# daooshee/ReReVST-Code

Hardware: AMD Instinct MI355X
Metric: stylized frames/sec at 512x512, 1 style (higher is better)
Workload: dtype f32

## Files before the change

rerevst-code_amd/csrc/conv_ups5.h:

```cpp
#pragma once

struct Ups5Tab {
    static constexpr int G2[5][3] = {{2, 0, 0}, {1, 1, 1}, {-1, -1, 1}, {-1, 1, 1}, {0, 0, 2}};
    static constexpr int BT4[4][4] = {{1, 0, -1, 0}, {0, 1, 1, 0}, {0, -1, 1, 0}, {0, -1, 0, 1}};
    static constexpr int AT[4][5] = {{1, 1, 0, -1, 0}, {0, 1, 1, 0, 0}, {0, 1, 0, 1, 0}, {0, 1, -1, 0, 1}};
    static constexpr int DS[5] = {0, 1, 2, 2, 3};
};
template <int T, int R>
constexpr int ups5_coef(int k) { return T == 0 ? Ups5Tab::BT4[R][k] : Ups5Tab::AT[R][k]; }
template <int T, int R, int N>
__device__ __forceinline__ f32x4 ups5_comb(const f32x4 (&x)[N]) {
    constexpr int F = [] { for (int k = 0; k < N; ++k) if (ups5_coef<T, R>(k) == 1) return k; return -1; }();
    static_assert(F >= 0, "every row has a +1 coefficient");
    f32x4 r = x[F];
    static_for([&](auto kc) {
        constexpr int k = decltype(kc)::value;
        constexpr int c = ups5_coef<T, R>(k);
        static_assert(c == 0 || c == 1 || c == -1, "0 / +-1 coefficients");
        if constexpr (k != F && c == 1) r = e4add(r, x[k]);
        else if constexpr (c == -1) r = f4sub(r, x[k]);
    }, std::make_integer_sequence<int, N>{});
    return r;
}

struct Ups5Geo {
    static constexpr int NT = 256, NB = 2;
    static constexpr int NPOS = 29;
    static constexpr int NUB = 26;
    static constexpr int NPIECE = 16;
    static constexpr int HALO = 18, HALF = 18 * 9;
    static constexpr int PIECES = HALO * HALO * 4;
    static constexpr int RAW_IT = (PIECES + NT - 1) / NT;
    static constexpr int RAW_BYTES = RAW_IT * NT * 16;
    static constexpr int U_BYTES = NUB * 32 * 16 * 4;
    static constexpr int U_IT = U_BYTES / 16 / NT;
    static_assert(U_IT * NT * 16 == U_BYTES, "U image is a whole number of LDS-DMA rounds");
    static constexpr int SMEM = 2 * RAW_BYTES + 2 * U_BYTES + WINO_PAR_BYTES;
    static_assert(SMEM <= 160 * 1024, "LDS");
    static constexpr int OCC = 1;
    static constexpr int vidx(int i) { return i < 25 ? Ups5Tab::DS[i % 5] * 4 + Ups5Tab::DS[i / 5] : (i == 25 ? 5 : i == 26 ? 9 : i == 27 ? 6 : 10); }
    static constexpr int issued(int j) { return (j + 2 < NUB ? 2 : 0) + (j < NPIECE ? 1 : 0); }
    static constexpr int younger(int i) {
        return i == 0 ? 2 + issued(0) : i == 1 ? issued(0) + issued(1) : (i - 2 < NPIECE ? 1 : 0) + issued(i - 1) + issued(i);
    }
    static constexpr int col_iter(int dx) { return 4 * dx + 6; }
    static constexpr int row_iter(int r) { return col_iter(3) + 1 + r; }
};
static_assert(Ups5Geo::row_iter(3) < Ups5Geo::NPOS, "next chunk transformed inside the MFMA loop");

template <int EPI, int PERIMG>
__device__ __forceinline__ void conv_ups5_body(const ConvP& p) {
    static_assert(!(EPI & (E_POOL | E_RES | E_RES_UPS | E_NORM2)), "conv1 epilogues only: bias, activation, saved-stat normalise");
    using G = Ups5Geo;
    constexpr int RAW_BYTES = G::RAW_BYTES, U_BYTES = G::U_BYTES, NT = G::NT, NB = G::NB, NPOS = G::NPOS, NUB = G::NUB;
    extern __shared__ __attribute__((aligned(16))) char smem[];
    const int tid = threadIdx.x;
    const int wave = __builtin_amdgcn_readfirstlane(tid >> 6);
    const int lane = tid & 63, t = lane & 15, q = lane >> 4;
    const int tr = t >> 3, tc = t & 7;
    const int tg = wave;
    const int nchunks = p.Cin >> 4;
    const int n_ntiles = p.Cout >> 5;

    struct Item { int tx, ty, b, nt; };
    Item cur, nxt, dlt;
    {
        const int GD = gridDim.x, w = blockIdx.x;
        int pix, dpix;
        if (p.xcd_slabs) {
            const int PT = (GD >> 3) / n_ntiles;
            pix = (w & 7) * PT + (w >> 3) / n_ntiles; dpix = 8 * PT;
            cur.nt = (w >> 3) % n_ntiles; dlt.nt = 0;
        } else {
            cur.nt = w % n_ntiles; pix = w / n_ntiles;
            dlt.nt = GD % n_ntiles; dpix = GD / n_ntiles;
        }
        cur.tx = pix % p.tiles_x; cur.ty = (pix / p.tiles_x) % p.tiles_y; cur.b = pix / (p.tiles_x * p.tiles_y);
        dlt.tx = dpix % p.tiles_x; dlt.ty = (dpix / p.tiles_x) % p.tiles_y; dlt.b = dpix / (p.tiles_x * p.tiles_y);
    }
    auto advance = [&](const Item& a) {
        Item r = a;
        r.nt += dlt.nt;
        int carry = 0;
        if (r.nt >= n_ntiles) { r.nt -= n_ntiles; carry = 1; }
        r.tx += dlt.tx + carry;
        if (r.tx >= p.tiles_x) { r.tx -= p.tiles_x; r.ty += 1; }
        r.ty += dlt.ty;
        if (r.ty >= p.tiles_y) { r.ty -= p.tiles_y; r.b += 1; }
        r.b += dlt.b;
        return r;
    };
    auto in_of = [&](const Item& a) {
        return p.in + (size_t)a.b * (size_t)(p.Hi + 2) * (p.Wi + 2) * p.Cin + (size_t)(((a.ty + p.ty0) * 16) * (p.Wi + 2) + (a.tx + p.tx0) * 16) * p.Cin;
    };
    auto w_of = [&](const Item& a) { return p.wpk + (size_t)a.nt * nchunks * (NUB * 32 * 16); };
    int asrc[G::RAW_IT];
#pragma unroll
    for (int it = 0; it < G::RAW_IT; ++it) {
        const int e = it * NT + tid;
        int P = e >> 2;
        const int qq = e & 3;
        if (P >= G::HALO * G::HALO) P = 0;
        const int hf = P >= G::HALF, rem = P - hf * G::HALF;
        const int hy = rem / 9, hx = 2 * (rem - hy * 9) + hf;
        asrc[it] = ((hy * (p.Wi + 2) + hx) * p.Cin + 4 * (qq ^ ((hx >> 1) & 3))) * 4;
    }
    const int raw_last_num = ((G::RAW_IT - 1) * NT + wave * 64 < G::PIECES) ? 0x7fffffff : 0;
    bool have = cur.b < p.B, have_nxt = false;
    const float* in_t = in_of(cur);
    const float* w_t = w_of(cur);
    const float* in_n = in_t;
    const float* w_n = w_t;
    auto stage_u = [&](int chunk) {
        char* udst = smem + 2 * RAW_BYTES + (chunk & 1) * U_BYTES;
#pragma unroll
        for (int it = 0; it < G::U_IT; ++it) bufld16(w_t, udst + (it * NT + wave * 64) * 16, tid * 16, chunk * U_BYTES + it * NT * 16);
    };
    auto stage_raw = [&](int chunk) {
        char* rdst = smem + (chunk & 1) * RAW_BYTES;
#pragma unroll
        for (int it = 0; it < G::RAW_IT; ++it)
            if (it * NT + wave * 64 < G::PIECES) bufld16(in_t, rdst + (it * NT + wave * 64) * 16, asrc[it], chunk * 64);
    };
    char* const par = smem + 2 * RAW_BYTES + 2 * U_BYTES;
    auto stage_params = [&](int ntile, int img) {
        if (wave < 2) {
            const int e = tid;
            const int row = e >> 3, col = (e & 7) * 4;
            const float* src = p.bias;
            const int pb = PERIMG ? img * p.par_bstride : 0;
            int off = ntile * 32 + col;
            if (row >= 1 && row <= 4) { src = (EPI & E_NORM1) ? p.n1 : p.bias; off = (EPI & E_NORM1) ? ntile * 32 + col + pb + (row - 1) * p.Cout : off; }
            if (row > 4) { src = p.bias; off = ntile * 32; }
            glds16(src + off, par + wave * 1024);
        }
    };

    const unsigned lds0 = (unsigned)(size_t)(__attribute__((address_space(3))) char*)smem;
    unsigned offD[4];
#pragma unroll
    for (int dx = 0; dx < 4; ++dx) {
        const int hy = 4 * tg + 2 * tr, hx = 2 * tc + dx;
        const int P = (hx & 1) * G::HALF + hy * 9 + (hx >> 1);
        offD[dx] = lds0 + P * 64 + ((q ^ ((hx >> 1) & 3)) << 4);
    }
    const unsigned offU = lds0 + 2 * RAW_BYTES + t * 64 + ((q ^ ((0 - (t >> 2)) & 3)) << 4);
    const unsigned offU1 = offU + U_BYTES;

    f32x4 acc[NPOS][NB];
    f32x4 va[16], vb[16];
    auto pass = [](f32x4& x0, f32x4& x1, f32x4& x2, f32x4& x3) {
        const f32x4 a[4] = {x0, x1, x2, x3};
        x0 = ups5_comb<0, 0>(a); x1 = ups5_comb<0, 1>(a); x2 = ups5_comb<0, 2>(a); x3 = ups5_comb<0, 3>(a);
    };
    auto col_pass = [&](f32x4 (&d)[16], int dx) { pass(d[dx * 4 + 0], d[dx * 4 + 1], d[dx * 4 + 2], d[dx * 4 + 3]); };
    auto row_pass = [&](f32x4 (&d)[16], int r) { pass(d[0 * 4 + r], d[1 * 4 + r], d[2 * 4 + r], d[3 * 4 + r]); };

    auto chunk_body = [&](int c, auto par_c, auto first_c, f32x4 (&vcur)[16], f32x4 (&vnext)[16]) {
        constexpr int PAR = decltype(par_c)::value;
        constexpr bool FIRST = decltype(first_c)::value;
        const bool own_u = c + 1 < nchunks, own_r = c + 2 < nchunks;
        const rsrc_t rs_u = make_rsrc(own_u ? w_t : w_n);
        const rsrc_t rs_r = make_rsrc(own_r ? in_t : in_n);
        const rsrc_t rs_rl = make_rsrc(own_r ? in_t : in_n, raw_last_num);
        const int usoff = own_u ? (c + 1) * U_BYTES : 0;
        const int rsoff = (own_r ? c + 2 : c + 2 - nchunks) * 64;
        char* const udst = smem + 2 * RAW_BYTES + (1 - PAR) * U_BYTES;
        char* const rdst = smem + PAR * RAW_BYTES;
        const unsigned ub = PAR ? offU1 : offU;
        constexpr int RB = (1 - PAR) * RAW_BYTES;
        f32x4 u[4][NB];
        f32x4 (&d)[16] = vnext;
        u[0][0] = lds_rd128<0>(ub);
        u[0][1] = lds_rd128<1024>(ub);
        u[1][0] = lds_rd128<2048>(ub);
        u[1][1] = lds_rd128<2048 + 1024>(ub);
        static_for([&](auto ic) {
            constexpr int i = decltype(ic)::value;
            if constexpr (i + 2 < NUB) {
                u[(i + 2) & 3][0] = lds_rd128<(i + 2) * 2048>(ub);
                u[(i + 2) & 3][1] = lds_rd128<(i + 2) * 2048 + 1024>(ub);
            }
            if constexpr (i < 16) d[i] = lds_rd128<RB + (i & 3) * 576>(offD[i >> 2]);
            constexpr int US = (i < NUB ? i : NUB - 1) & 3;
            if constexpr (i < NUB) {
                constexpr int cdx = (i - 6) / 4;
                if constexpr (i >= 6 && (i - 6) % 4 == 0 && cdx < 4) {
                    static_assert(G::col_iter(cdx) == i, "column release schedule");
                    asm volatile("s_waitcnt lgkmcnt(%6)" : "+v"(d[cdx * 4 + 0]), "+v"(d[cdx * 4 + 1]), "+v"(d[cdx * 4 + 2]), "+v"(d[cdx * 4 + 3]),
                                 "+v"(u[US][0]), "+v"(u[US][1]) : "i"(G::younger(i)));
                } else {
                    lds_release2<G::younger(i)>(u[US][0], u[US][1]);
                }
            }
            __builtin_amdgcn_sched_barrier(0);
            if constexpr (i < G::U_IT) bufld16_rs(rs_u, udst + (i * NT + wave * 64) * 16, tid * 16, usoff + i * NT * 16);
            if constexpr (i < G::RAW_IT) bufld16_rs(i == G::RAW_IT - 1 ? rs_rl : rs_r, rdst + (i * NT + wave * 64) * 16, asrc[i], rsoff);
            const f32x4 vv = vcur[G::vidx(i)];
#pragma unroll
            for (int s = 0; s < 4; ++s)
#pragma unroll
                for (int nb = 0; nb < NB; ++nb)
                    acc[i][nb] = __builtin_amdgcn_mfma_f32_16x16x4f32(u[US][nb][s], vv[s], (FIRST && s == 0) ? f32x4{0.f, 0.f, 0.f, 0.f} : acc[i][nb], 0, 0, 0);
            static_for([&](auto xc) {
                constexpr int k = decltype(xc)::value;
                if constexpr (G::col_iter(k) == i) col_pass(d, k);
                if constexpr (G::row_iter(k) == i) row_pass(d, k);
            }, std::make_integer_sequence<int, 4>{});
        }, std::make_integer_sequence<int, NPOS>{});
    };

    int par_ntile = -1, par_img = -1;
    if (have) {
        stage_raw(0);
        stage_u(0);
        stage_raw(1);
        stage_params(cur.nt, cur.b);
        par_ntile = cur.nt; par_img = cur.b;
        __syncthreads();
#pragma unroll
        for (int k = 0; k < 16; ++k) va[k] = *(const f32x4*)(smem + (offD[k >> 2] - lds0) + (k & 3) * 576);
#pragma unroll
        for (int dx = 0; dx < 4; ++dx) col_pass(va, dx);
#pragma unroll
        for (int r = 0; r < 4; ++r) row_pass(va, r);
        __syncthreads();
    }
    while (have) {
        const int e_y0 = (cur.ty + p.ty0) * 32, e_x0 = (cur.tx + p.tx0) * 32, e_b = cur.b, e_ntile = cur.nt;
        nxt = advance(cur);
        have_nxt = nxt.b < p.B;
        in_n = have_nxt ? in_of(nxt) : in_t;
        w_n = have_nxt ? w_of(nxt) : w_t;
        if (par_ntile != e_ntile || (PERIMG && par_img != e_b)) {
            __syncthreads();
            stage_params(e_ntile, e_b);
            par_ntile = e_ntile; par_img = e_b;
        }
        chunk_body(0, std::integral_constant<int, 0>{}, std::true_type{}, va, vb);
        __syncthreads();
        chunk_body(1, std::integral_constant<int, 1>{}, std::false_type{}, vb, va);
        __syncthreads();
        for (int c = 2; c < nchunks; c += 2) {
            chunk_body(c, std::integral_constant<int, 0>{}, std::false_type{}, va, vb);
            __syncthreads();
            chunk_body(c + 1, std::integral_constant<int, 1>{}, std::false_type{}, vb, va);
            __syncthreads();
        }
        cur = nxt; have = have_nxt; in_t = in_n; w_t = w_n;

        float* out_b = p.out + (size_t)e_b * (size_t)(p.H + 2) * (p.W + 2 + (p.out_p8 ? 6 : 0)) * p.Cout;
        const int yb = e_y0 + 8 * tg + 4 * tr, xb = e_x0 + 4 * tc;
        {
            const int ly0 = yb >> 1, lx0 = xb >> 1;
            float* sc_b = p.sc_out + (size_t)e_b * (size_t)(p.Hi + 2) * (p.Wi + 2) * p.Cout;
#pragma unroll
            for (int nb = 0; nb < NB; ++nb) {
                const f32x4 s0 = f4sub(acc[25][nb], acc[27][nb]), s1 = e4add(acc[25][nb], acc[27][nb]);
                const f32x4 t0 = f4sub(acc[26][nb], acc[28][nb]), t1 = e4add(acc[26][nb], acc[28][nb]);
                const f32x4 sc[2][2] = {{f4sub(s0, t0), e4add(s0, t0)}, {f4sub(s1, t1), e4add(s1, t1)}};
#pragma unroll
                for (int a = 0; a < 2; ++a)
#pragma unroll
                    for (int b = 0; b < 2; ++b) {
                        const int ly = ly0 + a, lx = lx0 + b;
                        if (ly < p.Hi && lx < p.Wi)
                            *(f32x4*)(sc_b + ((size_t)(ly + 1) * (p.Wi + 2) + lx + 1) * p.Cout + e_ntile * 32 + nb * 16 + 4 * q) = sc[a][b];
                    }
            }
        }
#pragma unroll
        for (int nb = 0; nb < NB; ++nb) {
            const int co = e_ntile * 32 + nb * 16 + 4 * q;
            f32x4 T[5][4];
#pragma unroll
            for (int r = 0; r < 5; ++r) {
                const f32x4 m[5] = {acc[r * 5 + 0][nb], acc[r * 5 + 1][nb], acc[r * 5 + 2][nb], acc[r * 5 + 3][nb], acc[r * 5 + 4][nb]};
                T[r][0] = ups5_comb<1, 0>(m); T[r][1] = ups5_comb<1, 1>(m); T[r][2] = ups5_comb<1, 2>(m); T[r][3] = ups5_comb<1, 3>(m);
            }
            f32x4 Y[4][4];
#pragma unroll
            for (int j = 0; j < 4; ++j) {
                const f32x4 tj[5] = {T[0][j], T[1][j], T[2][j], T[3][j], T[4][j]};
                Y[0][j] = ups5_comb<1, 0>(tj); Y[1][j] = ups5_comb<1, 1>(tj); Y[2][j] = ups5_comb<1, 2>(tj); Y[3][j] = ups5_comb<1, 3>(tj);
            }
            const char* pl = par + (nb * 16 + 4 * q) * 4;
            const f32x4 bias = *(const f32x4*)(pl);
            f32x4 m1, r1, lo1, hi1;
            if (EPI & E_NORM1) {
                m1 = *(const f32x4*)(pl + 128); r1 = *(const f32x4*)(pl + 256);
                lo1 = *(const f32x4*)(pl + 384); hi1 = *(const f32x4*)(pl + 512);
            }
#pragma unroll
            for (int i = 0; i < 4; ++i)
#pragma unroll
                for (int j = 0; j < 4; ++j) {
                    const int y = yb + i, x = xb + j;
                    f32x4 o = e4add(Y[i][j], bias);
                    if (EPI & E_RELU) o = f4relu(o);
                    if (EPI & E_LRELU) o = f4lrelu(o);
                    if (EPI & E_NORM1) o = f4norm_clamp(o, m1, r1, lo1, hi1);
                    if (y < p.H && x < p.W) {
                        if (p.out_p8) *(f32x4*)(out_b + (size_t)(co >> 3) * ((size_t)(p.H + 2) * (p.W + 8) * 8) + ((size_t)(y + 1) * (p.W + 8) + x + 4) * 8 + (co & 7)) = o;
                        else *(f32x4*)(out_b + ((size_t)(y + 1) * (p.W + 2) + x + 1) * p.Cout + co) = o;
                    }
                }
        }
    }
    asm volatile("s_waitcnt vmcnt(0)" ::: "memory");
}

__global__ void pack_ups5_k(const float* __restrict__ w, const float* __restrict__ wsc, float* __restrict__ dst, int Cout, int Cin) {
    constexpr int CH = 16, NUB = Ups5Geo::NUB;
    const size_t total = (size_t)Cout * Cin * NUB;
    for (size_t i = blockIdx.x * (size_t)blockDim.x + threadIdx.x; i < total; i += (size_t)gridDim.x * blockDim.x) {
        size_t r = i;
        const int cl = (int)(r % CH); r /= CH;
        const int j = r & 31; r >>= 5;
        const int pos = (int)(r % NUB); r /= NUB;
        const int nchunks = Cin / CH;
        const int chunk = r % nchunks; r /= nchunks;
        const int n_tile = (int)r;
        const int e = cl & 3, qs = cl >> 2;
        const int qq = qs ^ ((0 - (j >> 2)) & 3);
        const int co = n_tile * 32 + j, ci = chunk * CH + qq * 4 + e;
        if (pos == 25) { dst[i] = wsc[(size_t)co * Cin + ci] * 0.25f; continue; }
        const float* g = w + ((size_t)co * Cin + ci) * 9;
        auto G5 = [](int row, double g0, double g1, double g2) {
            return 0.5 * (Ups5Tab::G2[row][0] * g0 + Ups5Tab::G2[row][1] * g1 + Ups5Tab::G2[row][2] * g2);
        };
        const int pr = pos / 5, pc = pos % 5;
        double rowv[3];
#pragma unroll
        for (int kx = 0; kx < 3; ++kx) rowv[kx] = G5(pr, g[0 * 3 + kx], g[1 * 3 + kx], g[2 * 3 + kx]);
        dst[i] = (float)G5(pc, rowv[0], rowv[1], rowv[2]);
    }
}
```

rerevst-code_amd/csrc/conv_wino.h:

```cpp
#pragma once
#include <hip/hip_runtime.h>
#include <stdint.h>
#include <utility>
#include <type_traits>
#include "conv_mfma.h"

#define WINO_PAR_BYTES 2048

template <int NW, int UPS>
struct WinoGeo {
    static constexpr int NT = NW * 64;
    static constexpr int NB = NW == 8 ? 1 : 2;
    static constexpr int NP = UPS ? 9 : 16;
    static constexpr int NPU = NP;
    static constexpr int PW = UPS ? 3 : 4;
    static constexpr int NPIECE = PW * PW;
    static constexpr int PPI = UPS ? 3 : 2;
    static constexpr int TIN = UPS ? 8 : 16;
    static constexpr int HALO = UPS ? 10 : 18;
    static constexpr int HALF = 18 * 9;
    static constexpr int PIECES = HALO * HALO * 4;
    static constexpr int RAW_IT = (PIECES + NT - 1) / NT;
    static constexpr int RAW_BYTES = RAW_IT * NT * 16;
    static constexpr int U_BYTES = NPU * 32 * 16 * 4;
    static constexpr int U_PIECES = U_BYTES / 16;
    static constexpr int U_IT = (U_PIECES + NT - 1) / NT;
    static constexpr int U_LDS = U_IT * NT * 16;
    static constexpr int SMEM = 2 * RAW_BYTES + 2 * U_LDS + WINO_PAR_BYTES;
    static constexpr int OCC = (UPS && NW == 4) ? 2 : 1;
    static constexpr int col_iter(int dx) { return (dx * PW + PW - 1) / PPI + 3; }
    static constexpr int row_iter(int r) { return col_iter(PW - 1) + 1 + r; }
    static constexpr int pieces_in(int i) { return i < 0 ? 0 : (NPIECE - i * PPI <= 0 ? 0 : (NPIECE - i * PPI < PPI ? NPIECE - i * PPI : PPI)); }
    static constexpr int issued(int i) { return (i + 2 < NPU ? NB : 0) + pieces_in(i); }
    static constexpr int younger(int i) {
        return i == 0 ? NB + issued(0) : i == 1 ? issued(0) + issued(1) : pieces_in(i - 2) + issued(i - 1) + issued(i);
    }
};

template <int IMM>
__device__ __forceinline__ f32x4 lds_rd128(unsigned addr) {
    static_assert(IMM >= 0 && IMM < 65536, "ds_read offset is a 16-bit unsigned immediate");
    f32x4 r;
    asm volatile("ds_read_b128 %0, %1 offset:%2" : "=v"(r) : "v"(addr), "i"(IMM));
    return r;
}
template <int N>
__device__ __forceinline__ void lds_release1(f32x4& a) {
    asm volatile("s_waitcnt lgkmcnt(%1)" : "+v"(a) : "i"(N));
}
template <int N>
__device__ __forceinline__ void lds_release2(f32x4& a, f32x4& b) {
    asm volatile("s_waitcnt lgkmcnt(%2)" : "+v"(a), "+v"(b) : "i"(N));
}
template <int N>
__device__ __forceinline__ void lds_release3(f32x4& a, f32x4& b, f32x4& c) {
    asm volatile("s_waitcnt lgkmcnt(%3)" : "+v"(a), "+v"(b), "+v"(c) : "i"(N));
}
template <int N>
__device__ __forceinline__ void lds_release4(f32x4& a, f32x4& b, f32x4& c, f32x4& d) {
    asm volatile("s_waitcnt lgkmcnt(%4)" : "+v"(a), "+v"(b), "+v"(c), "+v"(d) : "i"(N));
}

__device__ __forceinline__ f32x4 f4sub(const f32x4 a, const f32x4 b) {
    typedef float f32x2 __attribute__((ext_vector_type(2)));
    f32x2 lo, hi;
    asm("v_pk_add_f32 %0, %1, %2 neg_lo:[0,1] neg_hi:[0,1]" : "=v"(lo) : "v"(__builtin_shufflevector(a, a, 0, 1)), "v"(__builtin_shufflevector(b, b, 0, 1)));
    asm("v_pk_add_f32 %0, %1, %2 neg_lo:[0,1] neg_hi:[0,1]" : "=v"(hi) : "v"(__builtin_shufflevector(a, a, 2, 3)), "v"(__builtin_shufflevector(b, b, 2, 3)));
    return __builtin_shufflevector(lo, hi, 0, 1, 2, 3);
}

__device__ __forceinline__ f32x4 f4add(const f32x4 a, const f32x4 b) {
    typedef float f32x2 __attribute__((ext_vector_type(2)));
    f32x2 lo, hi;
    asm("v_pk_add_f32 %0, %1, %2" : "=v"(lo) : "v"(__builtin_shufflevector(a, a, 0, 1)), "v"(__builtin_shufflevector(b, b, 0, 1)));
    asm("v_pk_add_f32 %0, %1, %2" : "=v"(hi) : "v"(__builtin_shufflevector(a, a, 2, 3)), "v"(__builtin_shufflevector(b, b, 2, 3)));
    return __builtin_shufflevector(lo, hi, 0, 1, 2, 3);
}

typedef float f32x2_t __attribute__((ext_vector_type(2)));
#define F4_LO(v) __builtin_shufflevector(v, v, 0, 1)
#define F4_HI(v) __builtin_shufflevector(v, v, 2, 3)
__device__ __forceinline__ f32x4 e4add(const f32x4 a, const f32x4 b) {
    const f32x2_t lo = F4_LO(a) + F4_LO(b), hi = F4_HI(a) + F4_HI(b);
    return __builtin_shufflevector(lo, hi, 0, 1, 2, 3);
}
__device__ __forceinline__ f32x4 e4mul(const f32x4 a, const f32x4 b) {
    const f32x2_t lo = F4_LO(a) * F4_LO(b), hi = F4_HI(a) * F4_HI(b);
    return __builtin_shufflevector(lo, hi, 0, 1, 2, 3);
}
__device__ __forceinline__ f32x4 e4fma(const f32x4 a, const f32x4 b, const f32x4 c) {
    const f32x2_t lo = __builtin_elementwise_fma(F4_LO(a), F4_LO(b), F4_LO(c)), hi = __builtin_elementwise_fma(F4_HI(a), F4_HI(b), F4_HI(c));
    return __builtin_shufflevector(lo, hi, 0, 1, 2, 3);
}
__device__ __forceinline__ float med3(float v, float lo, float hi) {
    float r;
    asm("v_med3_f32 %0, %1, %2, %3" : "=v"(r) : "v"(v), "v"(lo), "v"(hi));
    return r;
}
__device__ __forceinline__ f32x4 f4relu(f32x4 v) {
#pragma unroll
    for (int e = 0; e < 4; ++e) v[e] = fmaxf(v[e], 0.f);
    return v;
}
__device__ __forceinline__ f32x4 f4lrelu(const f32x4 v) {
    float k = 0.2f;
    asm volatile("" : "+s"(k));
    const f32x2_t k2 = {k, k};
    const f32x2_t lo = F4_LO(v) * k2, hi = F4_HI(v) * k2;
    const f32x4 s = __builtin_shufflevector(lo, hi, 0, 1, 2, 3);
    f32x4 r;
#pragma unroll
    for (int e = 0; e < 4; ++e) r[e] = fmaxf(v[e], s[e]);
    return r;
}
__device__ __forceinline__ f32x4 f4norm_clamp(const f32x4 v, const f32x4 m, const f32x4 r, const f32x4 lo, const f32x4 hi) {
    const f32x4 n = e4mul(f4sub(v, m), r);
    f32x4 o;
#pragma unroll
    for (int e = 0; e < 4; ++e) o[e] = med3(n[e], lo[e], hi[e]);
    return o;
}

template <class F, int... I>
__device__ __forceinline__ void static_for(F&& f, std::integer_sequence<int, I...>) {
    (f(std::integral_constant<int, I>{}), ...);
}

#include "conv_ups5.h"

template <int EPI, int ABL, int NW, int UPS, int PERIMG>
__device__ __forceinline__ void conv_upw_body(const ConvP& p) {
    static_assert(!(EPI & E_POOL), "no pooling behind an upsample");
    using G = WinoGeo<NW, UPS>;
    constexpr int NPU = G::NPU;
    constexpr int RAW_BYTES = G::RAW_BYTES, U_BYTES = G::U_BYTES, U_LDS = G::U_LDS, NT = G::NT, NB = G::NB, NP = G::NP, PW = G::PW, NPIECE = G::NPIECE;
    extern __shared__ __attribute__((aligned(16))) char smem[];
    const int tid = threadIdx.x;
    const int wave = __builtin_amdgcn_readfirstlane(tid >> 6);
    const int lane = tid & 63, t = lane & 15, q = lane >> 4;
    const int tr = t >> 3, tc = t & 7;
    const int tg = wave;
    const int nchunks = p.Cin >> 4;
    const int n_ntiles = p.Cout >> 5;

    struct Item { int tx, ty, b, nt; };
    Item cur, nxt, dlt;
    {
        const int GD = gridDim.x, w = blockIdx.x;
        int pix, dpix;
        if (p.xcd_slabs) {
            const int PT = (GD >> 3) / n_ntiles;
            pix = (w & 7) * PT + (w >> 3) / n_ntiles; dpix = 8 * PT;
            cur.nt = (w >> 3) % n_ntiles; dlt.nt = 0;
        } else {
            cur.nt = w % n_ntiles; pix = w / n_ntiles;
            dlt.nt = GD % n_ntiles; dpix = GD / n_ntiles;
        }
        cur.tx = pix % p.tiles_x; cur.ty = (pix / p.tiles_x) % p.tiles_y; cur.b = pix / (p.tiles_x * p.tiles_y);
        dlt.tx = dpix % p.tiles_x; dlt.ty = (dpix / p.tiles_x) % p.tiles_y; dlt.b = dpix / (p.tiles_x * p.tiles_y);
    }
    auto advance = [&](const Item& a) {
        Item r = a;
        r.nt += dlt.nt;
        int carry = 0;
        if (r.nt >= n_ntiles) { r.nt -= n_ntiles; carry = 1; }
        r.tx += dlt.tx + carry;
        if (r.tx >= p.tiles_x) { r.tx -= p.tiles_x; r.ty += 1; }
        r.ty += dlt.ty;
        if (r.ty >= p.tiles_y) { r.ty -= p.tiles_y; r.b += 1; }
        r.b += dlt.b;
        return r;
    };
    auto in_of = [&](const Item& a) {
        return p.in + (size_t)a.b * (size_t)(p.Hi + 2) * (p.Wi + 2) * p.Cin + (size_t)(((a.ty + p.ty0) * G::TIN) * (p.Wi + 2) + (a.tx + p.tx0) * G::TIN) * p.Cin;
    };
    auto w_of = [&](const Item& a) { return p.wpk + (size_t)a.nt * nchunks * (NPU * 32 * 16); };
    int asrc[G::RAW_IT];
#pragma unroll
    for (int it = 0; it < G::RAW_IT; ++it) {
        const int e = it * NT + tid;
        int P = e >> 2;
        const int qq = e & 3;
        if (P >= G::HALO * G::HALO) P = 0;
        const int hy = P / 10, hx = P - hy * 10, swz = hx & 3;
        asrc[it] = ((hy * (p.Wi + 2) + hx) * p.Cin + 4 * (qq ^ swz)) * 4;
    }
    const int raw_last_num = ((G::RAW_IT - 1) * NT + wave * 64 < G::PIECES) ? 0x7fffffff : 0;
    const int u_last_num = ((G::U_IT - 1) * NT + wave * 64 < G::U_PIECES) ? 0x7fffffff : 0;
    bool have = cur.b < p.B, have_nxt = false;
    const float* in_t = in_of(cur);
    const float* w_t = w_of(cur);
    const float* in_n = in_t;
    const float* w_n = w_t;
    auto stage_u = [&](int chunk) {
        char* udst = smem + 2 * RAW_BYTES + (chunk & 1) * U_LDS;
#pragma unroll
        for (int it = 0; it < G::U_IT; ++it)
            if (it * NT + wave * 64 < G::U_PIECES) bufld16(w_t, udst + (it * NT + wave * 64) * 16, tid * 16, chunk * U_BYTES + it * NT * 16);
    };
    auto stage_raw = [&](int chunk) {
        char* rdst = smem + (chunk & 1) * RAW_BYTES;
#pragma unroll
        for (int it = 0; it < G::RAW_IT; ++it)
            if (it * NT + wave * 64 < G::PIECES) bufld16(in_t, rdst + (it * NT + wave * 64) * 16, asrc[it], chunk * 64);
    };

    char* const par = smem + 2 * RAW_BYTES + 2 * U_LDS;
    auto stage_params = [&](int ntile, int img) {
        if (wave < 2) {
            const int e = tid;
            const int row = e >> 3, col = (e & 7) * 4;
            const float* src = p.bias;
            const int pb = PERIMG ? img * p.par_bstride : 0;
            int off = ntile * 32 + col;
            if (row >= 1 && row <= 4) { src = (EPI & E_NORM1) ? p.n1 : p.bias; off = (EPI & E_NORM1) ? ntile * 32 + col + pb + (row - 1) * p.Cout : off; }
            if (row >= 5 && row <= 8) { src = (EPI & E_NORM2) ? p.n2 : p.bias; off = (EPI & E_NORM2) ? ntile * 32 + col + pb + (row - 5) * p.Cout : off; }
            if (row >= 9) { src = (EPI & E_NORM2) ? p.sty : p.bias; off = (EPI & E_NORM2) ? ntile * 32 + col + pb + (row - 9) * p.Cout : off; }
            if (row > 10) { src = p.bias; off = ntile * 32; }
            glds16(src + off, par + wave * 1024);
        }
    };

    const unsigned lds0 = (unsigned)(size_t)(__attribute__((address_space(3))) char*)smem;
    unsigned offD[NPIECE];
#pragma unroll
    for (int dx = 0; dx < PW; ++dx)
#pragma unroll
        for (int dy = 0; dy < PW; ++dy) {
            const int hy = 2 * tg + tr + dy, hx = tc + dx;
            offD[dx * PW + dy] = lds0 + (hy * 10 + hx) * 64 + ((q ^ (hx & 3)) << 4);
        }
    const unsigned offU = lds0 + 2 * RAW_BYTES + t * 64 + ((q ^ ((0 - (t >> 2)) & 3)) << 4);
    const unsigned offU1 = offU + U_LDS;

    f32x4 acc[NPU][NB];
    f32x4 va[NPIECE], vb[NPIECE];
    auto pass = [](f32x4& d0, f32x4& d1, f32x4& d2) {
        const f32x4 a0 = d0, a1 = d1, a2 = d2;
        d0 = a1; d1 = f4sub(a0, a1); d2 = f4sub(a2, a1);
    };
    auto col_pass = [&](f32x4 (&d)[NPIECE], int dx) {
        pass(d[dx * PW + 0], d[dx * PW + 1], d[dx * PW + 2]);
    };
    auto row_pass = [&](f32x4 (&d)[NPIECE], int r) {
        pass(d[0 * PW + r], d[1 * PW + r], d[2 * PW + r]);
    };

    auto chunk_body = [&](int c, auto par_c, auto first_c, f32x4 (&vcur)[NPIECE], f32x4 (&vnext)[NPIECE]) {
        constexpr int PAR = decltype(par_c)::value;
        constexpr bool FIRST = decltype(first_c)::value;
        const bool own_u = c + 1 < nchunks, own_r = c + 2 < nchunks;
        const rsrc_t rs_u = make_rsrc(own_u ? w_t : w_n);
        const rsrc_t rs_ul = make_rsrc(own_u ? w_t : w_n, u_last_num);
        const rsrc_t rs_r = make_rsrc(own_r ? in_t : in_n);
        const rsrc_t rs_rl = make_rsrc(own_r ? in_t : in_n, raw_last_num);
        const int usoff = own_u ? (c + 1) * U_BYTES : 0;
        const int rsoff = (own_r ? c + 2 : c + 2 - nchunks) * 64;
        char* const udst = smem + 2 * RAW_BYTES + (1 - PAR) * U_LDS;
        char* const rdst = smem + PAR * RAW_BYTES;
        if (ABL & 128) {
            f32x4 u01[2] = {vcur[0], vcur[1]};
#pragma unroll
            for (int i = 0; i < NPU; ++i) {
                const f32x4 vv = vcur[i];
#pragma unroll
                for (int s = 0; s < 4; ++s)
#pragma unroll
                    for (int nb = 0; nb < NB; ++nb)
                        acc[i][nb] = __builtin_amdgcn_mfma_f32_16x16x4f32(u01[nb][s], vv[s], (FIRST && s == 0) ? f32x4{0.f, 0.f, 0.f, 0.f} : acc[i][nb], 0, 0, 0);
            }
#pragma unroll
            for (int i = 0; i < NPIECE; ++i) vnext[i] = vcur[i];
            return;
        }
        const unsigned ub = PAR ? offU1 : offU;
        constexpr int RB = (1 - PAR) * RAW_BYTES;
        f32x4 u[4][NB];
        f32x4 (&d)[NPIECE] = vnext;
        u[0][0] = lds_rd128<0>(ub);
        u[0][1] = lds_rd128<1024>(ub);
        u[1][0] = lds_rd128<2048>(ub);
        u[1][1] = lds_rd128<2048 + 1024>(ub);
        static_for([&](auto ic) {
            constexpr int i = decltype(ic)::value;
            if constexpr (i + 2 < NPU) {
                u[(i + 2) & 3][0] = lds_rd128<(i + 2) * 2048>(ub);
                u[(i + 2) & 3][1] = lds_rd128<(i + 2) * 2048 + 1024>(ub);
            }
            static_for([&](auto kc) {
                constexpr int pc = i * G::PPI + decltype(kc)::value;
                if constexpr (pc < NPIECE) d[pc] = lds_rd128<RB>(offD[pc]);
            }, std::make_integer_sequence<int, G::PPI>{});
            constexpr int cdx = i - 3;
            static_assert(G::col_iter(0) == 3 && G::col_iter(PW - 1) == PW + 2, "column release schedule");
            if constexpr (cdx >= 0 && cdx < PW) {
                asm volatile("s_waitcnt lgkmcnt(%5)" : "+v"(d[cdx * 3 + 0]), "+v"(d[cdx * 3 + 1]), "+v"(d[cdx * 3 + 2]), "+v"(u[i & 3][0]), "+v"(u[i & 3][1]) : "i"(G::younger(i)));
            } else {
                lds_release2<G::younger(i)>(u[i & 3][0], u[i & 3][1]);
            }
            __builtin_amdgcn_sched_barrier(0);
            if (!(ABL & 1)) {
                {
                    if constexpr (i < G::U_IT) bufld16_rs(i == G::U_IT - 1 ? rs_ul : rs_u, udst + (i * NT + wave * 64) * 16, tid * 16, usoff + i * NT * 16);
                    if constexpr (i < G::RAW_IT) bufld16_rs(i == G::RAW_IT - 1 ? rs_rl : rs_r, rdst + (i * NT + wave * 64) * 16, asrc[i], rsoff);
                }
            }
            const f32x4 vv = vcur[(i % PW) * PW + i / PW];
#pragma unroll
            for (int s = 0; s < 4; ++s)
#pragma unroll
                for (int nb = 0; nb < NB; ++nb)
                    acc[i][nb] = __builtin_amdgcn_mfma_f32_16x16x4f32(u[i & 3][nb][s], vv[s], (FIRST && s == 0) ? f32x4{0.f, 0.f, 0.f, 0.f} : acc[i][nb], 0, 0, 0);
            static_for([&](auto xc) {
                constexpr int k = decltype(xc)::value;
                if constexpr (G::col_iter(k) == i) col_pass(d, k);
                if constexpr (G::row_iter(k) == i) row_pass(d, k);
            }, std::make_integer_sequence<int, PW>{});
        }, std::make_integer_sequence<int, NPU>{});
    };

    int par_ntile = -1, par_img = -1;
    long long tl[6] = {0, 0, 0, 0, 0, 0}, tl_t = 0;
    auto tick = [&](int k) { if (ABL & 16) { const long long n = clock64(); tl[k] += n - tl_t; tl_t = n; } };
    if (ABL & 16) tl_t = clock64();
    if (have) {
        stage_raw(0);
        stage_u(0);
        stage_raw(1);
        stage_params(cur.nt, cur.b);
        par_ntile = cur.nt; par_img = cur.b;
        __syncthreads();
#pragma unroll
        for (int k = 0; k < NPIECE; ++k) va[k] = *(const f32x4*)(smem + (offD[k] - lds0));
#pragma unroll
        for (int dx = 0; dx < PW; ++dx) col_pass(va, dx);
#pragma unroll
        for (int r = 0; r < PW; ++r) row_pass(va, r);
        __syncthreads();
    }
    while (have) {
        const int e_y0 = (cur.ty + p.ty0) * 16, e_x0 = (cur.tx + p.tx0) * 16, e_b = cur.b, e_ntile = cur.nt;
        nxt = advance(cur);
        have_nxt = nxt.b < p.B;
        in_n = have_nxt ? in_of(nxt) : in_t;
        w_n = have_nxt ? w_of(nxt) : w_t;
        if (par_ntile != e_ntile || (PERIMG && par_img != e_b)) {
            __syncthreads();
            stage_params(e_ntile, e_b);
            par_ntile = e_ntile; par_img = e_b;
        }
        tick(0);
        chunk_body(0, std::integral_constant<int, 0>{}, std::true_type{}, va, vb);
        if (!(ABL & 2)) __syncthreads();
        chunk_body(1, std::integral_constant<int, 1>{}, std::false_type{}, vb, va);
        if (!(ABL & 2)) __syncthreads();
        for (int c = 2; c < nchunks; c += 2) {
            chunk_body(c, std::integral_constant<int, 0>{}, std::false_type{}, va, vb);
            if (!(ABL & 2)) __syncthreads();
            chunk_body(c + 1, std::integral_constant<int, 1>{}, std::false_type{}, vb, va);
            if (!(ABL & 2)) __syncthreads();
        }
        tick(3);
        cur = nxt; have = have_nxt; in_t = in_n; w_t = w_n;
        if constexpr ((ABL & 32) != 0) {
            f32x4 sacc = acc[0][0];
#pragma unroll
            for (int i = 0; i < NPU; ++i)
#pragma unroll
                for (int nb = 0; nb < NB; ++nb) if (i || nb) sacc += acc[i][nb];
            if (sacc[0] + sacc[1] + sacc[2] + sacc[3] == 123.456f) p.out[tid] = sacc[0];
            continue;
        }
        float* out_b = p.out + (size_t)e_b * (size_t)(p.H + 2) * (p.W + 2 + (p.out_p8 ? 6 : 0)) * p.Cout;
        const float* res_b = nullptr;
        if (EPI & (E_RES | E_RES_UPS)) res_b = p.res + (size_t)e_b * (size_t)(p.Hr + 2) * (p.Wr + 2) * p.Cout;
        const int yb = e_y0 + 4 * tg + 2 * tr, xb = e_x0 + 2 * tc;
        f32x4 resv[NB][2][2];
        if (EPI & (E_RES | E_RES_UPS)) {
#pragma unroll
            for (int nb = 0; nb < NB; ++nb)
#pragma unroll
                for (int i = 0; i < 2; ++i)
#pragma unroll
                    for (int j = 0; j < 2; ++j) {
                        const int y = yb + i, x = xb + j;
                        const int ry = (EPI & E_RES_UPS) ? (y >> 1) : y, rx = (EPI & E_RES_UPS) ? (x >> 1) : x;
                        resv[nb][i][j] = f32x4{0.f, 0.f, 0.f, 0.f};
                        if (y < p.H && x < p.W)
                            resv[nb][i][j] = *(const f32x4*)(res_b + ((ry + 1) * (p.Wr + 2) + rx + 1) * p.Cout + e_ntile * 32 + nb * 16 + 4 * q);
                    }
        }
#pragma unroll
        for (int nb = 0; nb < NB; ++nb) {
            const int co = e_ntile * 32 + nb * 16 + 4 * q;
            f32x4 Y[2][2];
            f32x4 T[2][3];
#pragma unroll
            for (int c = 0; c < 3; ++c) {
                T[0][c] = acc[0 + c][nb] + acc[3 + c][nb];
                T[1][c] = acc[0 + c][nb] + acc[6 + c][nb];
            }
#pragma unroll
            for (int i = 0; i < 2; ++i) {
                Y[i][0] = T[i][0] + T[i][1];
                Y[i][1] = T[i][0] + T[i][2];
            }
            const char* pl = par + (nb * 16 + 4 * q) * 4;
            const f32x4 bias = *(const f32x4*)(pl);
            f32x4 m1, r1, lo1, hi1, m2, r2, lo2, hi2, smean, sstd;
            if (EPI & E_NORM1) {
                m1 = *(const f32x4*)(pl + 128); r1 = *(const f32x4*)(pl + 256);
                lo1 = *(const f32x4*)(pl + 384); hi1 = *(const f32x4*)(pl + 512);
            }
            if (EPI & E_NORM2) {
                m2 = *(const f32x4*)(pl + 640); r2 = *(const f32x4*)(pl + 768);
                lo2 = *(const f32x4*)(pl + 896); hi2 = *(const f32x4*)(pl + 1024);
                smean = *(const f32x4*)(pl + 1152); sstd = *(const f32x4*)(pl + 1280);
            }
#pragma unroll
            for (int i = 0; i < 2; ++i)
#pragma unroll
                for (int j = 0; j < 2; ++j) {
                    const int y = yb + i, x = xb + j;
                    f32x4 o = e4add(Y[i][j], bias);
                    if (EPI & E_RELU) o = f4relu(o);
                    if (EPI & E_LRELU) o = f4lrelu(o);
                    if (EPI & E_NORM1) o = f4norm_clamp(o, m1, r1, lo1, hi1);
                    if (EPI & (E_RES | E_RES_UPS)) o = e4add(o, resv[nb][i][j]);
                    if (EPI & E_NORM2) o = e4fma(f4norm_clamp(o, m2, r2, lo2, hi2), sstd, smean);
                    if (y < p.H && x < p.W) {
                        if (ABL & 4) { if (o[0] == 123.456f) out_b[co] = o[0]; }
                        else if (p.out_p8) *(f32x4*)(out_b + (size_t)(co >> 3) * ((size_t)(p.H + 2) * (p.W + 8) * 8) + ((size_t)(y + 1) * (p.W + 8) + x + 4) * 8 + (co & 7)) = o;
                        else *(f32x4*)(out_b + ((y + 1) * (p.W + 2) + x + 1) * p.Cout + co) = o;
                    }
                }
        }
        tick(5);
    }
    asm volatile("s_waitcnt vmcnt(0)" ::: "memory");
    if ((ABL & 16) && lane == 0) {
        long long* dbg = p.dbg;
#pragma unroll
        for (int k = 0; k < 6; ++k) dbg[(blockIdx.x * NW + wave) * 6 + k] = tl[k];
    }
}

template <int EPI, int ABL = 0, int NW = 4, int UPS = 1, int SC = 0, int PERIMG = 0>
__global__ __launch_bounds__(NW * 64, (SC ? Ups5Geo::OCC : WinoGeo<NW, UPS>::OCC)) void conv_wino_k(const ConvP p) {
    static_assert(UPS == 1 && NW == 4, "library kernel: upsample-fused form, 4 waves");
    if constexpr (SC) conv_ups5_body<EPI, PERIMG>(p);
    else conv_upw_body<EPI, ABL, NW, UPS, PERIMG>(p);
}

__global__ void pack_wino_k(const float* __restrict__ w, float* __restrict__ dst, int Cout, int Cin, int ups) {
    constexpr int CH = 16;
    const int npt = ups ? 9 : 16, pw = ups ? 3 : 4;
    const int np = npt;
    const size_t total = (size_t)Cout * Cin * np;
    for (size_t i = blockIdx.x * (size_t)blockDim.x + threadIdx.x; i < total; i += (size_t)gridDim.x * blockDim.x) {
        size_t r = i;
        const int cl = (int)(r % CH); r /= CH;
        const int j = r & 31; r >>= 5;
        const int pos = (int)(r % np); r /= np;
        const int nchunks = Cin / CH;
        const int chunk = r % nchunks; r /= nchunks;
        const int n_tile = (int)r;
        const int e = cl & 3, qs = cl >> 2;
        const int qq = qs ^ ((0 - (j >> 2)) & 3);
        const int co = n_tile * 32 + j, ci = chunk * CH + qq * 4 + e;
        const float* g = w + ((size_t)co * Cin + ci) * 9;
        const int pr = pos / pw, pc = pos % pw;
        auto G3 = [&](int row, float g0, float g1, float g2) {
            if (ups) return row == 0 ? g0 + g1 + g2 : (row == 1 ? g0 : g2);
            return row == 0 ? g0 : (row == 1 ? 0.5f * (g0 + g1 + g2) : (row == 2 ? 0.5f * (g0 - g1 + g2) : g2));
        };
        float rowv[3];
#pragma unroll
        for (int kx = 0; kx < 3; ++kx) rowv[kx] = G3(pr, g[0 * 3 + kx], g[1 * 3 + kx], g[2 * 3 + kx]);
        dst[i] = G3(pc, rowv[0], rowv[1], rowv[2]);
    }
}
```

Baseline: 857.7.

## Transpose ups5 MFMA output and pack epilogue as paired f32x2 ops

Swaps the MFMA operand order so each lane holds accumulators for output pixels across two channel pairs, and reorders packed weight channels to match (co = 2*(j&15)+(j>>4)). The epilogue then runs the Winograd output transform, bias, activation and normalisation on f32x2 vectors using packed adds and subtracts, writing 8-byte stores with precomputed base offsets. A fast path skips bounds checks on interior tiles. It also adds optional clock64 timing probes and an ablation flag, both off by default. The aim is fewer epilogue instructions and cheaper address math, at the cost of narrower stores and a changed weight layout.

```diff
diff --git a/rerevst-code_amd/csrc/conv_ups5.h b/rerevst-code_amd/csrc/conv_ups5.h
--- a/rerevst-code_amd/csrc/conv_ups5.h
+++ b/rerevst-code_amd/csrc/conv_ups5.h
@@ -8,21 +8,33 @@
 };
 template <int T, int R>
 constexpr int ups5_coef(int k) { return T == 0 ? Ups5Tab::BT4[R][k] : Ups5Tab::AT[R][k]; }
-template <int T, int R, int N>
-__device__ __forceinline__ f32x4 ups5_comb(const f32x4 (&x)[N]) {
+__device__ __forceinline__ f32x4 ups5_add(const f32x4 a, const f32x4 b) { return e4add(a, b); }
+__device__ __forceinline__ f32x4 ups5_sub(const f32x4 a, const f32x4 b) { return f4sub(a, b); }
+__device__ __forceinline__ f32x2_t ups5_add(const f32x2_t a, const f32x2_t b) { return a + b; }
+__device__ __forceinline__ f32x2_t ups5_sub(const f32x2_t a, const f32x2_t b) {
+    f32x2_t r;
+    asm("v_pk_add_f32 %0, %1, %2 neg_lo:[0,1] neg_hi:[0,1]" : "=v"(r) : "v"(a), "v"(b));
+    return r;
+}
+template <int T, int R, class V, int N>
+__device__ __forceinline__ V ups5_comb(const V (&x)[N]) {
     constexpr int F = [] { for (int k = 0; k < N; ++k) if (ups5_coef<T, R>(k) == 1) return k; return -1; }();
     static_assert(F >= 0, "every row has a +1 coefficient");
-    f32x4 r = x[F];
+    V r = x[F];
     static_for([&](auto kc) {
         constexpr int k = decltype(kc)::value;
         constexpr int c = ups5_coef<T, R>(k);
         static_assert(c == 0 || c == 1 || c == -1, "0 / +-1 coefficients");
-        if constexpr (k != F && c == 1) r = e4add(r, x[k]);
-        else if constexpr (c == -1) r = f4sub(r, x[k]);
+        if constexpr (k != F && c == 1) r = ups5_add(r, x[k]);
+        else if constexpr (c == -1) r = ups5_sub(r, x[k]);
     }, std::make_integer_sequence<int, N>{});
     return r;
 }
 
+#ifndef P8_PAD
+#define P8_PAD 6
+#define P8_COL0 4
+#endif
 struct Ups5Geo {
     static constexpr int NT = 256, NB = 2;
     static constexpr int NPOS = 29;
@@ -48,7 +60,7 @@
 };
 static_assert(Ups5Geo::row_iter(3) < Ups5Geo::NPOS, "next chunk transformed inside the MFMA loop");
 
-template <int EPI, int PERIMG>
+template <int EPI, int ABL, int PERIMG>
 __device__ __forceinline__ void conv_ups5_body(const ConvP& p) {
     static_assert(!(EPI & (E_POOL | E_RES | E_RES_UPS | E_NORM2)), "conv1 epilogues only: bias, activation, saved-stat normalise");
     using G = Ups5Geo;
@@ -201,16 +213,19 @@
             for (int s = 0; s < 4; ++s)
 #pragma unroll
                 for (int nb = 0; nb < NB; ++nb)
-                    acc[i][nb] = __builtin_amdgcn_mfma_f32_16x16x4f32(u[US][nb][s], vv[s], (FIRST && s == 0) ? f32x4{0.f, 0.f, 0.f, 0.f} : acc[i][nb], 0, 0, 0);
+                    acc[i][nb] = __builtin_amdgcn_mfma_f32_16x16x4f32(vv[s], u[US][nb][s], (FIRST && s == 0) ? f32x4{0.f, 0.f, 0.f, 0.f} : acc[i][nb], 0, 0, 0);
             static_for([&](auto xc) {
                 constexpr int k = decltype(xc)::value;
-                if constexpr (G::col_iter(k) == i) col_pass(d, k);
-                if constexpr (G::row_iter(k) == i) row_pass(d, k);
+                if constexpr (!(ABL & 8) && G::col_iter(k) == i) col_pass(d, k);
+                if constexpr (!(ABL & 8) && G::row_iter(k) == i) row_pass(d, k);
             }, std::make_integer_sequence<int, 4>{});
         }, std::make_integer_sequence<int, NPOS>{});
     };
 
     int par_ntile = -1, par_img = -1;
+    long long tl[6] = {0, 0, 0, 0, 0, 0}, tl_t = 0;
+    auto tick = [&](int k) { if (ABL & 16) { const long long n = clock64(); tl[k] += n - tl_t; tl_t = n; } };
+    auto chunk_barrier = [&]() { tick(1); __syncthreads(); tick(3); };
     if (have) {
         stage_raw(0);
         stage_u(0);
@@ -226,6 +241,7 @@
         for (int r = 0; r < 4; ++r) row_pass(va, r);
         __syncthreads();
     }
+    if (ABL & 16) tl_t = clock64();
     while (have) {
         const int e_y0 = (cur.ty + p.ty0) * 32, e_x0 = (cur.tx + p.tx0) * 32, e_b = cur.b, e_ntile = cur.nt;
         nxt = advance(cur);
@@ -237,75 +253,112 @@
             stage_params(e_ntile, e_b);
             par_ntile = e_ntile; par_img = e_b;
         }
+        tick(0);
         chunk_body(0, std::integral_constant<int, 0>{}, std::true_type{}, va, vb);
-        __syncthreads();
+        chunk_barrier();
         chunk_body(1, std::integral_constant<int, 1>{}, std::false_type{}, vb, va);
-        __syncthreads();
+        chunk_barrier();
         for (int c = 2; c < nchunks; c += 2) {
             chunk_body(c, std::integral_constant<int, 0>{}, std::false_type{}, va, vb);
-            __syncthreads();
+            chunk_barrier();
             chunk_body(c + 1, std::integral_constant<int, 1>{}, std::false_type{}, vb, va);
-            __syncthreads();
+            chunk_barrier();
         }
         cur = nxt; have = have_nxt; in_t = in_n; w_t = w_n;
 
-        float* out_b = p.out + (size_t)e_b * (size_t)(p.H + 2) * (p.W + 2 + (p.out_p8 ? 6 : 0)) * p.Cout;
-        const int yb = e_y0 + 8 * tg + 4 * tr, xb = e_x0 + 4 * tc;
-        {
-            const int ly0 = yb >> 1, lx0 = xb >> 1;
-            float* sc_b = p.sc_out + (size_t)e_b * (size_t)(p.Hi + 2) * (p.Wi + 2) * p.Cout;
-#pragma unroll
-            for (int nb = 0; nb < NB; ++nb) {
-                const f32x4 s0 = f4sub(acc[25][nb], acc[27][nb]), s1 = e4add(acc[25][nb], acc[27][nb]);
-                const f32x4 t0 = f4sub(acc[26][nb], acc[28][nb]), t1 = e4add(acc[26][nb], acc[28][nb]);
-                const f32x4 sc[2][2] = {{f4sub(s0, t0), e4add(s0, t0)}, {f4sub(s1, t1), e4add(s1, t1)}};
-#pragma unroll
-                for (int a = 0; a < 2; ++a)
-#pragma unroll
-                    for (int b = 0; b < 2; ++b) {
-                        const int ly = ly0 + a, lx = lx0 + b;
-                        if (ly < p.Hi && lx < p.Wi)
-                            *(f32x4*)(sc_b + ((size_t)(ly + 1) * (p.Wi + 2) + lx + 1) * p.Cout + e_ntile * 32 + nb * 16 + 4 * q) = sc[a][b];
-                    }
-            }
-        }
-#pragma unroll
-        for (int nb = 0; nb < NB; ++nb) {
-            const int co = e_ntile * 32 + nb * 16 + 4 * q;
-            f32x4 T[5][4];
+        const int mr = q >> 1, mc = q & 1;
+        const int yb = e_y0 + 8 * tg + 4 * mr, xb0 = e_x0 + 16 * mc;
+        char* sb;
+        int rowb, pixb;
+        unsigned st_off;
+        if (p.out_p8) {
+            const int WP = p.W + 2 + P8_PAD;
+            const unsigned plane = (unsigned)(p.H + 2) * WP * 32u;
+            sb = (char*)(p.out + (size_t)e_b * (size_t)(p.H + 2) * WP * p.Cout + (size_t)e_ntile * 4 * (size_t)(p.H + 2) * WP * 8 +
+                         ((size_t)(e_y0 + 8 * tg + 1) * WP + e_x0 + P8_COL0) * 8);
+            rowb = WP * 32; pixb = 32;
+            st_off = (unsigned)(4 * mr * WP + 16 * mc) * 32u + (unsigned)(t >> 2) * plane + (unsigned)(t & 3) * 8u;
+        } else {
+            sb = (char*)(p.out + (size_t)e_b * (size_t)(p.H + 2) * (p.W + 2) * p.Cout + ((size_t)(e_y0 + 8 * tg + 1) * (p.W + 2) + e_x0 + 1) * p.Cout + e_ntile * 32);
+            rowb = (p.W + 2) * p.Cout * 4; pixb = p.Cout * 4;
+            st_off = (unsigned)((4 * mr * (p.W + 2) + 16 * mc) * p.Cout + 2 * t) * 4u;
+        }
+        char* const scb = (char*)(p.sc_out + (size_t)e_b * (size_t)(p.Hi + 2) * (p.Wi + 2) * p.Cout +
+                                  ((size_t)((e_y0 >> 1) + 4 * tg + 1) * (p.Wi + 2) + (e_x0 >> 1) + 1) * p.Cout + e_ntile * 32);
+        const int sc_rowb = (p.Wi + 2) * p.Cout * 4, sc_pixb = p.Cout * 4;
+        const unsigned sc_off = (unsigned)((2 * mr * (p.Wi + 2) + 8 * mc) * p.Cout + 2 * t) * 4u;
+        const bool interior = e_y0 + 32 <= p.H && e_x0 + 32 <= p.W;
+        const char* const pl = par + 8 * t;
+        const f32x2_t bias = *(const f32x2_t*)(pl);
+        f32x2_t n1m, n1r, n1lo, n1hi;
+        if constexpr ((EPI & E_NORM1) != 0) { n1m = *(const f32x2_t*)(pl + 128); n1r = *(const f32x2_t*)(pl + 256); n1lo = *(const f32x2_t*)(pl + 384); n1hi = *(const f32x2_t*)(pl + 512); }
+        float lrk = 0.2f;
+        asm volatile("" : "+s"(lrk));
+        const f32x2_t lrk2 = {lrk, lrk};
+#pragma unroll
+        for (int e = 0; e < 4; ++e) {
+            auto PR = [&](int i) -> f32x2_t { return f32x2_t{acc[i][0][e], acc[i][1][e]}; };
+            {
+                const f32x2_t p25 = PR(25), p26 = PR(26), p27 = PR(27), p28 = PR(28);
+                const f32x2_t s0 = ups5_sub(p25, p27), s1 = ups5_add(p25, p27);
+                const f32x2_t t0 = ups5_sub(p26, p28), t1 = ups5_add(p26, p28);
+                const f32x2_t sc[2][2] = {{ups5_sub(s0, t0), ups5_add(s0, t0)}, {ups5_sub(s1, t1), ups5_add(s1, t1)}};
+                char* const dst = scb + (2 * e) * sc_pixb + sc_off;
+                if (interior) {
+#pragma unroll
+                    for (int a = 0; a < 2; ++a)
+#pragma unroll
+                        for (int b = 0; b < 2; ++b) *(f32x2_t*)(dst + a * sc_rowb + b * sc_pixb) = sc[a][b];
+                } else {
+#pragma unroll
+                    for (int a = 0; a < 2; ++a)
+#pragma unroll
+                        for (int b = 0; b < 2; ++b)
+                            if ((yb >> 1) + a < p.Hi && ((xb0 + 4 * e) >> 1) + b < p.Wi) *(f32x2_t*)(dst + a * sc_rowb + b * sc_pixb) = sc[a][b];
+                }
+            }
+            f32x2_t T[5][4];
 #pragma unroll
             for (int r = 0; r < 5; ++r) {
-                const f32x4 m[5] = {acc[r * 5 + 0][nb], acc[r * 5 + 1][nb], acc[r * 5 + 2][nb], acc[r * 5 + 3][nb], acc[r * 5 + 4][nb]};
+                const f32x2_t m[5] = {PR(r * 5 + 0), PR(r * 5 + 1), PR(r * 5 + 2), PR(r * 5 + 3), PR(r * 5 + 4)};
                 T[r][0] = ups5_comb<1, 0>(m); T[r][1] = ups5_comb<1, 1>(m); T[r][2] = ups5_comb<1, 2>(m); T[r][3] = ups5_comb<1, 3>(m);
             }
-            f32x4 Y[4][4];
 #pragma unroll
             for (int j = 0; j < 4; ++j) {
-                const f32x4 tj[5] = {T[0][j], T[1][j], T[2][j], T[3][j], T[4][j]};
-                Y[0][j] = ups5_comb<1, 0>(tj); Y[1][j] = ups5_comb<1, 1>(tj); Y[2][j] = ups5_comb<1, 2>(tj); Y[3][j] = ups5_comb<1, 3>(tj);
-            }
-            const char* pl = par + (nb * 16 + 4 * q) * 4;
-            const f32x4 bias = *(const f32x4*)(pl);
-            f32x4 m1, r1, lo1, hi1;
-            if (EPI & E_NORM1) {
-                m1 = *(const f32x4*)(pl + 128); r1 = *(const f32x4*)(pl + 256);
-                lo1 = *(const f32x4*)(pl + 384); hi1 = *(const f32x4*)(pl + 512);
-            }
-#pragma unroll
-            for (int i = 0; i < 4; ++i)
-#pragma unroll
-                for (int j = 0; j < 4; ++j) {
-                    const int y = yb + i, x = xb + j;
-                    f32x4 o = e4add(Y[i][j], bias);
-                    if (EPI & E_RELU) o = f4relu(o);
-                    if (EPI & E_LRELU) o = f4lrelu(o);
-                    if (EPI & E_NORM1) o = f4norm_clamp(o, m1, r1, lo1, hi1);
-                    if (y < p.H && x < p.W) {
-                        if (p.out_p8) *(f32x4*)(out_b + (size_t)(co >> 3) * ((size_t)(p.H + 2) * (p.W + 8) * 8) + ((size_t)(y + 1) * (p.W + 8) + x + 4) * 8 + (co & 7)) = o;
-                        else *(f32x4*)(out_b + ((size_t)(y + 1) * (p.W + 2) + x + 1) * p.Cout + co) = o;
-                    }
-                }
-        }
+                const f32x2_t tj[5] = {T[0][j], T[1][j], T[2][j], T[3][j], T[4][j]};
+                f32x2_t o[4] = {ups5_comb<1, 0>(tj), ups5_comb<1, 1>(tj), ups5_comb<1, 2>(tj), ups5_comb<1, 3>(tj)};
+#pragma unroll
+                for (int i = 0; i < 4; ++i) o[i] = o[i] + bias;
+                if (EPI & E_RELU) {
+#pragma unroll
+                    for (int i = 0; i < 4; ++i) o[i] = f32x2_t{fmaxf(o[i][0], 0.f), fmaxf(o[i][1], 0.f)};
+                }
+                if (EPI & E_LRELU) {
+#pragma unroll
+                    for (int i = 0; i < 4; ++i) { const f32x2_t s2 = o[i] * lrk2; o[i] = f32x2_t{fmaxf(o[i][0], s2[0]), fmaxf(o[i][1], s2[1])}; }
+                }
+                if constexpr ((EPI & E_NORM1) != 0) {
+#pragma unroll
+                    for (int i = 0; i < 4; ++i) o[i] = ups5_sub(o[i], n1m) * n1r;
+#pragma unroll
+                    for (int i = 0; i < 4; ++i) o[i] = f32x2_t{med3(o[i][0], n1lo[0], n1hi[0]), med3(o[i][1], n1lo[1], n1hi[1])};
+                }
+                char* const dst = sb + (4 * e + j) * pixb + st_off;
+                if (interior) {
+#pragma unroll
+                    for (int i = 0; i < 4; ++i) *(f32x2_t*)(dst + i * rowb) = o[i];
+                } else {
+#pragma unroll
+                    for (int i = 0; i < 4; ++i)
+                        if (yb + i < p.H && xb0 + 4 * e + j < p.W) *(f32x2_t*)(dst + i * rowb) = o[i];
+                }
+            }
+        }
+        tick(4);
+    }
+    if ((ABL & 16) && lane == 0) {
+#pragma unroll
+        for (int k = 0; k < 6; ++k) p.dbg[(blockIdx.x * 4 + wave) * 6 + k] = tl[k];
     }
     asm volatile("s_waitcnt vmcnt(0)" ::: "memory");
 }
@@ -323,7 +376,7 @@
         const int n_tile = (int)r;
         const int e = cl & 3, qs = cl >> 2;
         const int qq = qs ^ ((0 - (j >> 2)) & 3);
-        const int co = n_tile * 32 + j, ci = chunk * CH + qq * 4 + e;
+        const int co = n_tile * 32 + 2 * (j & 15) + (j >> 4), ci = chunk * CH + qq * 4 + e;
         if (pos == 25) { dst[i] = wsc[(size_t)co * Cin + ci] * 0.25f; continue; }
         const float* g = w + ((size_t)co * Cin + ci) * 9;
         auto G5 = [](int row, double g0, double g1, double g2) {
diff --git a/rerevst-code_amd/csrc/conv_wino.h b/rerevst-code_amd/csrc/conv_wino.h
--- a/rerevst-code_amd/csrc/conv_wino.h
+++ b/rerevst-code_amd/csrc/conv_wino.h
@@ -448,7 +448,7 @@
 template <int EPI, int ABL = 0, int NW = 4, int UPS = 1, int SC = 0, int PERIMG = 0>
 __global__ __launch_bounds__(NW * 64, (SC ? Ups5Geo::OCC : WinoGeo<NW, UPS>::OCC)) void conv_wino_k(const ConvP p) {
     static_assert(UPS == 1 && NW == 4, "library kernel: upsample-fused form, 4 waves");
-    if constexpr (SC) conv_ups5_body<EPI, PERIMG>(p);
+    if constexpr (SC) conv_ups5_body<EPI, ABL, PERIMG>(p);
     else conv_upw_body<EPI, ABL, NW, UPS, PERIMG>(p);
 }
 
```

Result: no change. 858.4, median of 2 (+0.1%).
